# TopAY-Planner/TopAY

Hardware: AMD Instinct MI355X
Metric: trajectories/sec to L-BFGS convergence (benchmark_tables batch) at 1/2/4/8 GPU (higher is better)
Workload: dtype f64

## Files before the change

include/topay.h:

```cpp
#ifndef TOPAY_H
#define TOPAY_H

#include <stdint.h>

#ifdef __cplusplus
extern "C" {
#endif

typedef int topay_status;
enum {
  TOPAY_OK = 0,
  TOPAY_ERR_INVALID_ARG = -1,
  TOPAY_ERR_NO_DEVICE = -2,
  TOPAY_ERR_NO_MAP = -3,
  TOPAY_ERR_NO_TRAJ = -4,
  TOPAY_ERR_TOO_MANY_PIECES = -5,
  TOPAY_ERR_UNSUPPORTED = -6
};

enum {
  TOPAY_LBFGS_CONVERGENCE = 0,
  TOPAY_LBFGS_STOP = 1,
  TOPAY_LBFGS_CANCELED = 2,
  TOPAY_LBFGSERR_INVALID_FUNCVAL = -1012,
// ... 215 lines not shown

topay_status topay_set_latency_mode(topay_ctx* ctx, int mode);

typedef struct { char internal[128]; } topay_comm_id_t;
typedef struct {
  int scenario_id;
  int best_candidate;
  int status;
  int n_pieces;
  double cost;
  double duration;
} topay_record_t;
topay_status topay_comm_unique_id(topay_comm_id_t* id);
topay_status topay_comm_init(topay_ctx* ctx, const topay_comm_id_t* id, int world, int rank);
topay_status topay_comm_destroy(topay_ctx* ctx);
topay_status topay_scenario_records(topay_ctx* ctx, const int* scenario_of, int cap_records, topay_record_t* records, int* n_records,
                                    int* winner_index);
topay_status topay_gather_records(topay_ctx* ctx, const topay_record_t* mine, int n_mine, int per_rank, topay_record_t* all, int* n_valid);
topay_status topay_pack_records(const topay_record_t* mine, int n_mine, int per_rank, topay_record_t* block);
topay_status topay_unpack_records(const topay_record_t* gathered, int world, int per_rank, topay_record_t* all, int* n_valid);

topay_status topay_class_of(int n_pieces, int* waves, int* elements_per_thread, int* class_index);

topay_status topay_workspace_bytes(topay_ctx* ctx, unsigned long long* bytes);

topay_status topay_gate_timeouts(topay_ctx* ctx, int* n);

topay_status topay_last_kernel_ms(topay_ctx* ctx, double* ms, int* launches);
topay_status topay_last_helper_launches(topay_ctx* ctx, int* n);

#ifdef __cplusplus
}
#endif
#endif
```

topay_amd/csrc/topay_eval.h:

```cpp
#pragma once

#include <hip/hip_runtime.h>

#include "topay_math.h"
#include "topay_types.h"

#ifndef TOPAY_CPU_EMU
#define HIP_DYN_SHARED_DECL extern __shared__ double topay_lds[];
#endif

__constant__ DevParams g_P;
typedef const TOPAY_CST DevParams& dev_params_ref;
__device__ __forceinline__ dev_params_ref dev_params() {
#ifndef TOPAY_CPU_EMU
  const TOPAY_CST DevParams* p = (const TOPAY_CST DevParams*)&g_P;
  asm("" : "+s"(p));
  return *p;
#else
  return g_P;
#endif
}

#ifdef TOPAY_USE_SCHED_FENCE
#define TOPAY_SCHED_FENCE() __builtin_amdgcn_sched_barrier(0)
// ... 352 lines not shown
  gx = g0 * ri;
  dist = q.in ? dist : 0.0; gx = q.in ? gx : 0.0; gy = q.in ? gy : 0.0; gz = q.in ? gz : 0.0;
}

struct EvalCtx {
  int lane, N, rows, n;
  int tid, wave;
  lds_dp red;
  lds_dp adj;
  glb_dp coefg;
  int cl_in_lds;
  lds_dp cL;
  lds_dp Tp;
  glb_cdp hd, tl;
  int npass_lds;
  lds_dp gdT;
  lds_dp pcs;
  lds_dp gC;
  glb_dp sbuf;
  int sb_stride;
  glb_dp mstash;
  lds_dp pw;
  lds_dp X;
  glb_cdp x;
  glb_dp g;
  glb_dp lu;
  glb_cdp init_xy;
  double sx, sy, ex, ey;
  double lam0, lam1, rho0, rho1;
  double fxe0, fxe1;
  TOPAY_GLB long long* stamps;
  long long t_last;
};

__device__ __forceinline__ void fill_power_table(lds_dp pw, int lane) {
  for (int t = lane; t < 156; t += 64) {
    const int jj = t / 6, k = t - 6 * jj;
    double v = 1.0;
    for (int u = 0; u < k; u++) v *= (double)jj;
    pw[t] = v;
  }
}

#define BAND(i, j) band[((i) - (j) + 6) * rows + (j)]

#ifdef TOPAY_STAMPS
// ... 14 lines not shown
  } while (0)
#else
#define SUBSTAMP_BEGIN(C) do { } while (0)
#define SUBSTAMP_END(C, k) do { } while (0)
#endif

struct GradGate {
  bool always;
  bool has_early;
  double finit, thr , early ;
  bool early_ok;
  double skip_thr;
  __device__ __forceinline__ bool needs(double f) const {
    if (always) return true;
    if (isinf(f) || isnan(f)) return false;
    if (has_early && fabs(finit - f) / (fabs(finit) + 1.0) < early) return true;
    return !(f > thr);
  }
};

#define TOPAY_SWEEP_CHUNK 24
#define TOPAY_SWEEP_WCOLS 30
#define TOPAY_SWEEP_WIN (7 * TOPAY_SWEEP_WCOLS)
template <int MODE>
__device__ __forceinline__ void band_sweep(lds_dp v, bool owner, glb_cdp lu, lds_dp win, int rows, int lane) {
  constexpr bool FWD = (MODE == 0 || MODE == 2);
  constexpr bool SCALE = (MODE == 1 || MODE == 2);
  constexpr int D0 = (MODE == 0 || MODE == 3) ? 7 : 0;
  constexpr int CH = TOPAY_SWEEP_CHUNK, WC = TOPAY_SWEEP_WCOLS, WIN = TOPAY_SWEEP_WIN;
  constexpr int NEL = (SCALE ? 7 : 6) * WC;
  constexpr int NQ = (NEL + 63) / 64;
  double w[6];
  double x = 0.0;
#pragma unroll
  for (int t = 0; t < 6; t++) w[t] = 0.0;
  if (owner) {
    if (FWD) {
      x = v[0];
#pragma unroll
      for (int t = 0; t < 6; t++) w[t] = v[1 + t];
    } else {
      x = v[rows - 1];
#pragma unroll
      for (int t = 0; t < 6; t++) w[t] = v[rows - 2 - t];
    }
  }
  const int nchunk = (rows + CH - 1) / CH;
  auto chunk_clo = [&](int k) { return FWD ? CH * k : rows - 1 - CH * k - (WC - 1); };
  auto request = [&](int k, double (&q)[NQ]) {
    const int clo = chunk_clo(k);
#pragma unroll
    for (int u = 0; u < NQ; u++) {
      const int e = lane + 64 * u;
      const int r = e / WC, cc = e - r * WC;
      int c = clo + cc;
      c = c < 0 ? 0 : (c > rows - 1 ? rows - 1 : c);
      const int d = (r < 6 ? D0 + r : 13);
      q[u] = lu[(d < 14 ? d : 13) * rows + c];
    }
  };
  auto deposit = [&](int k, const double (&q)[NQ]) {
    lds_dp wb = win + (k & 1) * WIN;
#pragma unroll
    for (int u = 0; u < NQ; u++) {
      const int e = lane + 64 * u;
      if (e < NEL) wb[e] = q[u];
    }
  };
// ... 554 lines not shown
```

topay_amd/csrc/topay_eval_mw.h:

```cpp
#pragma once
#include "topay_eval.h"

namespace topay {

__device__ __forceinline__ void wg_lds_barrier() {
#ifndef TOPAY_CPU_EMU
  __builtin_amdgcn_fence(__ATOMIC_RELEASE, "workgroup", "local");
  __builtin_amdgcn_s_barrier();
  __builtin_amdgcn_fence(__ATOMIC_ACQUIRE, "workgroup", "local");
#else
  __syncthreads();
#endif
}

template <int NW>
__device__ __forceinline__ void wg_barrier() {
  if (NW == 1) lds_sync();
  else wg_lds_barrier();
}

template <int NW>
__device__ __forceinline__ void wg_global_barrier() {
  if (NW == 1) lds_sync();
  else __syncthreads();
// ... 21 lines not shown
  lds_dp r = red + (phase & 1) * 4;
  phase++;
  r[wave] = wm;
  wg_lds_barrier();
  double m = r[0] > r[1] ? r[0] : r[1];
  if (NW == 4) {
    const double m2 = r[2] > r[3] ? r[2] : r[3];
    m = m > m2 ? m : m2;
  }
  return m;
}

__host__ __device__ __forceinline__ int mw_pb_rows(int NW) { return NW == 1 ? 7 : 14; }
__host__ __device__ __forceinline__ int mw_npass(int Nmax) { return (TOPAY_EP * Nmax + 63) / 64; }
__host__ __device__ __forceinline__ int mw_red_doubles(int NW) { return NW > 1 ? 8 : 0; }
__host__ __device__ __forceinline__ int mw_misc_doubles(int Nmax, int NW) {
  return mw_red_doubles(NW) + 2 * mw_npass(Nmax) + (NW > 1 ? 2 * NW * 64 : 0) + NW;
}
__host__ __device__ __forceinline__ int lds_doubles_mw(int Nmax, int NW) {
  const int rows = 6 * Nmax;
  const int lu = 14 * rows, sw = 9 * rows + 26 * Nmax + mw_pb_rows(NW) * 64 * NW;
  return 5 * Nmax + Nmax + 4 * (Nmax + 1) + 156 + mw_misc_doubles(Nmax, NW) + (lu > sw ? lu : sw);
}
__device__ __forceinline__ void carve_mw(EvalCtx& C, lds_dp base, int Nmax, int NW) {
  const int rows = 6 * Nmax;
  lds_dp p = base;
  C.Tp = p; p += 5 * Nmax;
  C.gdT = p; p += Nmax;
  C.pcs = p; p += 4 * (Nmax + 1);
  C.pw = p; p += 156;
  C.red = p; p += mw_misc_doubles(Nmax, NW);
  C.cL = p;
  C.adj = C.cL;
  C.gC = C.adj;
  C.X = p + 9 * rows;
  C.npass_lds = mw_npass(Nmax);
}

template <int NW, int OCC>
__device__ __noinline__ void minco_generate_mw(EvalCtx& C) {
  constexpr int NT = 64 * NW;
  const lds_dp c_Tp = C.Tp;
  const lds_dp c_X = C.X;
  const lds_dp c_gdT = C.gdT;
  const glb_cdp c_hd = C.hd, c_tl = C.tl;
  const glb_dp c_lu = C.lu;
  const glb_cdp c_x = C.x;
  dev_params_ref P = dev_params();
  const int tid = C.tid, lane = C.lane, wave = __builtin_amdgcn_readfirstlane(C.wave);
  const int N = __builtin_amdgcn_readfirstlane(C.N), rows = __builtin_amdgcn_readfirstlane(C.rows);
  lds_dp cL = C.cL;
  lds_dp band = cL;
  lds_dp rdiag = cL + 13 * rows;
  glb_cdp Tau = c_x;
  glb_cdp Theta = c_x + N;
  glb_cdp Arc = c_x + 2 * N - 1;
  glb_cdp Vq = c_x + 3 * N - 1;

  const double tau_v = tid < N ? Tau[tid] : 0.0;
  constexpr int NI = 9;
  double inner_v[NI];
#pragma unroll
  for (int u = 0; u < NI; u++) {
    const int t = tid + NT * u;
    inner_v[u] = 0.0;
    if (t < 9 * (N - 1)) {
      const int i = t / 9, d = t - 9 * i;
      const int dq = d >= 2 ? d - 2 : 0;
      inner_v[u] = d == 0 ? Theta[i] : (d == 1 ? Arc[i] : Vq[i * 7 + dq]);
    }
  }
  double bc_v[6] = {0.0, 0.0, 0.0, 0.0, 0.0, 0.0};
  if (tid < 9) {
    const int d = tid;
    bc_v[0] = c_hd[0 * 9 + d]; bc_v[1] = c_hd[1 * 9 + d]; bc_v[2] = c_hd[2 * 9 + d];
    bc_v[3] = (d == 1) ? Arc[N - 1] : c_tl[0 * 9 + d];
// ... 40 lines not shown
  if (wave == 0) {
    const int t = lane / 7 + 1, u = lane - (lane / 7) * 7;
    const bool lane_in = lane < 42;
    const int o_kk = 6 * rows;
    const int o_ik = lane_in ? (t + 6) * rows : o_kk;
    const int o_ij = lane_in ? (t - u + 6) * rows + u : o_kk;
    const int o_kj = lane_in ? (6 - u) * rows + u : o_kk;
    for (int k = 0; k <= rows - 2; k++) {
      const int i = k + t, j = k + u;
      const bool act = lane_in && (i < rows) && (j < rows);
      double akk = band[o_kk + k], aik = band[o_ik + k], aij = band[o_ij + k], akj = band[o_kj + k];
      TOPAY_OPAQUE(aij); TOPAY_OPAQUE(akj);
      const double m = aik / akk;
      const double nv = (u == 0) ? m : (aij - m * akj);
      lds_sync();
      if (act) band[o_ij + k] = nv;
      lds_sync();
    }
  }
  wg_barrier<NW>();
  STAMP(C, 1);
  for (int t = tid; t < rows; t += NT) rdiag[t] = 1.0 / BAND(t, t);
  wg_barrier<NW>();
  for (int t = tid; t < 14 * rows; t += NT) c_lu[t] = band[t];
  if (NW == 1) lds_sync();
  else { wave_global_sync(); wg_barrier<NW>(); }
  for (int t = tid; t < 9 * rows; t += NT) cL[t] = 0.0;
  wg_barrier<NW>();
  if (tid < 9) {
    const int d = tid;
    cL[d * rows + 0] = bc_v[0];
    cL[d * rows + 1] = bc_v[1];
    cL[d * rows + 2] = bc_v[2];
    cL[d * rows + rows - 3] = bc_v[3];
    cL[d * rows + rows - 2] = bc_v[4];
    cL[d * rows + rows - 1] = bc_v[5];
  }
#pragma unroll
  for (int u = 0; u < NI; u++) {
    const int t = tid + NT * u;
    if (t < 9 * (N - 1)) {
      const int i = t / 9, d = t - 9 * i;
      const int dq = d >= 2 ? d - 2 : 0;
      cL[d * rows + 6 * i + 5] = d >= 2 ? sigmoidC2(inner_v[u], P.joint_pos_limit_max[dq]) : inner_v[u];
    }
  }
  wg_barrier<NW>();
  if (wave == 0) {
    const bool owner = lane < 9;
    const lds_dp mine = cL + (owner ? lane : 8) * rows;
    band_sweep<0>(mine, owner, (glb_cdp)c_lu, c_X, rows, lane);
    band_sweep<1>(mine, owner, (glb_cdp)c_lu, c_X, rows, lane);
  }
  C.cl_in_lds = 1;
  wg_barrier<NW>();
  STAMP(C, 2);
}

template <int STAGE, int RMAX, int NW, int OCC = 1>
__device__ __noinline__ TOPAY_CALLS_BIG_FUNCTIONS double eval_cost_grad_mw(EvalCtx& C, const TOPAY_GLB DevMap* mp, const GradGate gate) {
  constexpr int NT = 64 * NW;
  const lds_dp c_Tp = uniform_ptr(C.Tp);
  const lds_dp c_X = uniform_ptr(C.X);
  const double c_ex = uniform_f64(C.ex);
  const double c_ey = uniform_f64(C.ey);
  const glb_dp c_g = uniform_ptr(C.g);
  const lds_dp c_gdT = uniform_ptr(C.gdT);
  const glb_cdp c_init_xy = uniform_ptr(C.init_xy);
  const double c_lam0 = uniform_f64(C.lam0);
  const double c_lam1 = uniform_f64(C.lam1);
  const glb_dp c_lu = uniform_ptr(C.lu);
  const lds_dp c_pcs = uniform_ptr(C.pcs);
  const lds_dp c_pw = uniform_ptr(C.pw);
  const double c_rho0 = uniform_f64(C.rho0);
  const double c_rho1 = uniform_f64(C.rho1);
// ... 6 lines not shown

  dev_params_ref P = dev_params();
  int lane = C.lane, tid = C.tid;
  const int wave = __builtin_amdgcn_readfirstlane(C.wave);
  const int N = __builtin_amdgcn_readfirstlane(C.N), rows = __builtin_amdgcn_readfirstlane(C.rows);
  lds_cdp cL = uniform_ptr(C.cL);
  const glb_dp c_sbuf = uniform_ptr(C.sbuf);
  const glb_dp c_mstash = uniform_ptr(C.mstash);
  const int c_sbs = __builtin_amdgcn_readfirstlane(C.sb_stride);
  const double g_skip_thr = uniform_f64(gate.skip_thr);
  const bool g_early_ok = __builtin_amdgcn_readfirstlane(gate.early_ok ? 1 : 0) != 0;
  GradGate ugate;
  ugate.always = __builtin_amdgcn_readfirstlane(gate.always ? 1 : 0) != 0;
  ugate.has_early = __builtin_amdgcn_readfirstlane(gate.has_early ? 1 : 0) != 0;
  ugate.finit = uniform_f64(gate.finit); ugate.thr = uniform_f64(gate.thr); ugate.early = uniform_f64(gate.early);
  ugate.early_ok = g_early_ok; ugate.skip_thr = g_skip_thr;
  int rp = 0;
  const int npl = __builtin_amdgcn_readfirstlane(C.npass_lds);
  constexpr int RD = NW > 1 ? 8 : 0;
  const lds_dp ptot = c_red + RD;
  const lds_dp csr = c_red + RD + 2 * npl;
  TOPAY_LDS unsigned long long* jmask = (TOPAY_LDS unsigned long long*)(c_red + RD + 2 * npl + (NW > 1 ? 2 * NW * 64 : 0));
  constexpr int PBR = NW == 1 ? 7 : 14;
  minco_generate_mw<NW, OCC>(C);

  auto jerk_terms = [&](int i, double& e_out, double& gdT_out) __attribute__((always_inline)) {
    double w33 = 0, w43 = 0, w44 = 0, w53 = 0, w54 = 0, w55 = 0;
#pragma unroll
    for (int d = 0; d < 9; d++) {
      const double c3 = cL[d * rows + 6 * i + 3], c4 = cL[d * rows + 6 * i + 4], c5 = cL[d * rows + 6 * i + 5];
      const double e = P.energy_weights[d];
      w33 += (c3 * e) * c3; w43 += (c4 * e) * c3; w44 += (c4 * e) * c4;
      w53 += (c5 * e) * c3; w54 += (c5 * e) * c4; w55 += (c5 * e) * c5;
    }
    const double T1 = c_Tp[i], T2 = c_Tp[N + i], T3 = c_Tp[2 * N + i], T4 = c_Tp[3 * N + i], T5 = c_Tp[4 * N + i];
    e_out = 36.0 * w33 * T1 + 144.0 * w43 * T2 + 192.0 * w44 * T3 + 240.0 * w53 * T3 + 720.0 * w54 * T4 + 720.0 * w55 * T5;
    gdT_out = 36.0 * w33 + 288.0 * w43 * T1 + 576.0 * w44 * T2 + 720.0 * w53 * T2 + 2880.0 * w54 * T3 + 3600.0 * w55 * T4;
  };
  double jerk_e = 0.0;
  if (tid < N) {
    double unused_;
    jerk_terms(tid, jerk_e, unused_);
  }
  const double jerk_cost = wg_sum<NW>(c_red, rp, wave, jerk_e);

  lds_dp gxy = c_X;
// ... 79 lines not shown
        posy = c_sy + (carryy + py0);
      };
      geometry(lane);
      if (act && m == TOPAY_K) {
        c_pcs[2 * N + 2 * (i + 1)] = posx;
        c_pcs[2 * N + 2 * (i + 1) + 1] = posy;
      }
      if (!skip_body) {
        ManiOut mo;
        mo.gx = mo.gy = mo.gth = mo.cost = mo.gdT = 0.0;
        if (STAGE == 2) {
          mo = sample_mani<OCC>(cL, rows, i, j, e, act, step, half, posx, posy, mp, c_mstash, pbuf + lane);
          lane = fresh_lane_id(lane);
          tid = wave * 64 + lane;
          geometry(lane);
        }
        double gB[12], gdTs, gpx, gpy, cst;
        bool jva;
        sample_rest<STAGE>(P, cL, rows, i, j, step, half, posx, posy, mp, wM, wA, wD, mo, pbuf + lane, gB, gdTs, gpx, gpy, jva, cst);
        if (act) {
          cst_out = cst;
          gxy[2 * e] = gpx;
          gxy[2 * e + 1] = gpy;
          glb_dp sb = c_sbuf + e;
          const int ss = c_sbs;
#pragma unroll
          for (int v = 0; v < 5; v++) sb[v * ss] = gB[v];
          sb[5 * ss] = gdTs;
          if (STAGE == 2) {
#pragma unroll
            for (int v = 0; v < 7; v++) sb[(6 + v) * ss] = gB[5 + v];
            sb[13 * ss] = jva ? 1.0 : 0.0;
          }
        }
      }
    }
    lds_dp cs = csr + (k & 1) * (NW * 64);
    if (NW > 1) {
      cs[wave * 64 + lane] = cst_out;
      wg_barrier<NW>();
    }
#pragma unroll
    for (int q = 0; q < NW; q++) {
      const int p2 = k * NW + q;
      if (p2 < npass) {
        cost_pen += NW > 1 ? cs[q * 64 + lane] : cst_out;
        if (STAGE == 2 && g_early_ok && !skip_body && p2 + 1 < npass) {
          const double partial = jerk_cost + wave_sum(cost_pen) + time_cost;
          if (partial > g_skip_thr && partial <= 1.79769313486231570e308) {
            skip_body = true;
            f_skip = partial;
          }
        }
      }
    }
// ... 74 lines not shown
  for (int r = 0; r < RMAX; r++) {
    a0[r] = 0.0;
    a1[r] = 0.0;
#pragma unroll
    for (int q = 0; q < 7; q++) aq[r][q] = 0.0;
    rbh[r][0] = rbh[r][1] = rbh[r][2] = 0.0;
    if (ract[r]) {
      const double hs = c_Tp[rpiece[r]] / TOPAY_K / 2.0;
      basis_k(rk[r], hs, rbh[r][0], rbh[r][1], rbh[r][2]);
    }
  }
  constexpr int NV = (STAGE == 2) ? 13 : 6;
  if constexpr (NW == 1) {
    for (int pass = 0; pass < npass; pass++) {
      const int e = pass * 64 + lane;
      const bool act = e < NE;
      const int i = act ? e / TOPAY_EP : N - 1;
      const int m = act ? e - TOPAY_EP * i : 0;
      const int j = 2 * m;
      const double step = c_Tp[i] / TOPAY_K, half = step / 2.0;
      bool jva = false;
      double rawq[7];
      {
        glb_cdp sb = c_sbuf + (act ? e : NE - 1);
        const int ss = c_sbs;
        double raw[14];
#pragma unroll
        for (int v = 0; v < ((STAGE == 2) ? 14 : 6); v++) raw[v] = sb[v * ss];
#pragma unroll
        for (int v = 0; v < 6; v++) pbuf[v * 64 + lane] = act ? raw[v] : 0.0;
#pragma unroll
        for (int v = 0; v < 7; v++) rawq[v] = (STAGE == 2 && act) ? raw[6 + v] : 0.0;
        if (STAGE == 2) jva = act && raw[13] != 0.0;
      }
      lds_sync();
#pragma unroll
      for (int r = 0; r < RMAX; r++) {
        if (ract[r]) {
          const int pi = rpiece[r];
          const double h0 = rbh[r][0], h1 = rbh[r][1], h2 = rbh[r][2];
          const int k0 = rk[r], k1 = rk[r] >= 1 ? rk[r] - 1 : 0, k2 = rk[r] >= 2 ? rk[r] - 2 : 0;
          const int e_lo = max(TOPAY_EP * pi, pass * 64), e_hi = min(min(TOPAY_EP * pi + TOPAY_EP, pass * 64 + 64), NE);
          double gt = 0.0;
          constexpr int CH = 3;
          for (int c0 = e_lo; c0 < e_hi; c0 += CH) {
            double pb[CH][6], t0[CH], t1[CH], t2[CH];
#pragma unroll
            for (int u = 0; u < CH; u++) {
              const int ee = (c0 + u < e_hi) ? c0 + u : e_hi - 1;
              const int l = ee - pass * 64, mm = ee - TOPAY_EP * pi;
              lds_cdp pj = c_pw + 12 * mm;
// ... 401 lines not shown
          const double e = P.energy_weights[d];
          if (kk == 5) jg = 240.0 * c3 * e * T3 + 720.0 * c4 * e * T4 + 1440.0 * c5 * e * T5;
          else if (kk == 4) jg = 144.0 * c3 * e * T2 + 384.0 * c4 * e * T3 + 720.0 * c5 * e * T4;
          else jg = 72.0 * c3 * e * T1 + 144.0 * c4 * e * T2 + 240.0 * c5 * e * T3;
        }
        tot[r][d] = jg + (d == 0 ? a0[r] : (d == 1 ? a1[r] : aq[r][d >= 2 ? d - 2 : 0]));
      }
    }
  }
  for (int t = tid; t < 9 * rows; t += NT) c_coefg[t] = cL[t];
  C.cl_in_lds = 0;
  wg_global_barrier<NW>();
#pragma unroll
  for (int r = 0; r < RMAX; r++) {
    if (ract[r]) {
#pragma unroll
      for (int d = 0; d < 9; d++) c_adj[d * rows + rrow[r]] = tot[r][d];
    }
  }
  wg_barrier<NW>();
  if (wave == 0) {
    const bool owner = lane < 9;
    const lds_dp mine = c_adj + (owner ? lane : 8) * rows;
    band_sweep<2>(mine, owner, (glb_cdp)c_lu, c_X, rows, lane);
    band_sweep<3>(mine, owner, (glb_cdp)c_lu, c_X, rows, lane);
  }
  wg_barrier<NW>();
  STAMP(C, 7);
#pragma unroll
  for (int r = 0; r < RMAX; r++) {
    if (ract[r]) {
      const int row = rrow[r];
      int pi, br;
      bool use = true;
      if (row >= rows - 3) { pi = N - 1; br = 10 + (row - (rows - 3)); }
      else if (row < 3) { use = false; pi = 0; br = 0; }
      else { pi = (row - 3) / 6; br = (row - 3) - 6 * pi; }
      double part = 0.0;
      if (use) {
        const double T1 = c_Tp[pi], T2 = c_Tp[N + pi], T3 = c_Tp[2 * N + pi], T4 = c_Tp[3 * N + pi];
#pragma unroll
        for (int d = 0; d < 9; d++) {
          glb_cdp cg = c_coefg + d * rows + 6 * pi;
          const double c1 = cg[1], c2 = cg[2], c3 = cg[3], c4 = cg[4], c5 = cg[5];
          double b;
          if (br == 0) b = -(24.0 * c4 + 120.0 * T1 * c5);
          else if (br == 1) b = -120.0 * c5;
          else if (br == 2 || br == 3 || br == 10) b = -(c1 + 2.0 * T1 * c2 + 3.0 * T2 * c3 + 4.0 * T3 * c4 + 5.0 * T4 * c5);
// ... 36 lines not shown
```

topay_amd/csrc/topay_hip.hip:

```cpp
#include <hip/hip_runtime.h>

#include <algorithm>
#include <cstdio>
#include <cstdint>
#include <cstring>
#include <numeric>
#include <cstdlib>
#include <chrono>
#include <cmath>
#include <mutex>
#include <thread>
#include <string>
#include <vector>
#include <dlfcn.h>

#include "topay_solve.h"
#include "topay_feas.h"
#include "topay_edt.h"
#include "topay_front.h"
#include "topay_mcrrt.h"
#include "topay_jps.h"
#include "topay_topo.h"
#include "topay_yaml.h"

// ... 94 lines not shown
      if (atoi(e) == 4) {
        if (w4 == 4) t[4] = {42, 2, 4, k_solve2w4, k_eval2w4, 2};
        if (w5 == 4) t[5] = {64, 2, 4, k_solve2w4, k_eval2w4, 2};
        t[6] = {128, 3, 4, k_solve3w4, k_eval3w4, 2};
      }
    }
#endif
    return t;
  }();
  return tab;
}
static const int kLdsDoublesPerCU = 160 * 1024 / 8;
static size_t class_lds_bytes(const ClassDef& cd, int nm) {
  int d = lds_doubles_mw(nm, cd.nw);
  if (const char* e = exp_env("TOPAY_LDS_PAD")) {
    for (const char* q = e; q && *q;) {
      int mn = 0, add = 0;
      if (sscanf(q, "%d:%d", &mn, &add) == 2 && mn == cd.max_n) d += add;
      q = strchr(q, ',');
      if (q) q++;
    }
  }
  return (size_t)(d + 8 + 40 + (cd.helpers ? TOPAY_CMD_DOUBLES : 0)) * sizeof(double);
}

__attribute__((constructor)) static void topay_request_hw_queues() { setenv("GPU_MAX_HW_QUEUES", "24", 0); }
struct topay_ctx;
static std::mutex g_issue_mutex;
static std::mutex g_registry_mutex;
static std::vector<topay_ctx*> g_contexts;

static topay_ctx* g_last_issued = nullptr;

struct topay_ctx {
  int device = 0;
  topay_params_t hp;
  DevParams dp;
  hipStream_t stream = nullptr;
  hipEvent_t ev0 = nullptr, ev1 = nullptr;
  std::vector<DevMap> hmaps = std::vector<DevMap>(TOPAY_MAX_MAPS);
  std::vector<DevBuf> map2d = std::vector<DevBuf>(TOPAY_MAX_MAPS), map3d = std::vector<DevBuf>(TOPAY_MAX_MAPS);
  std::vector<DevBuf> map2d_inf = std::vector<DevBuf>(TOPAY_MAX_MAPS), map2d_crit = std::vector<DevBuf>(TOPAY_MAX_MAPS);
  struct MapArena { DevBuf buf; int first = 0, n = 0; };
  std::vector<MapArena> map_arenas;
  DevBuf dmaps;
  std::vector<char> have_map = std::vector<char>(TOPAY_MAX_MAPS, 0);
// ... 10 lines not shown
  std::vector<int> cls[NBUCKET];
  hipStream_t bstream[NBUCKET] = {nullptr};
  hipEvent_t bevent[NBUCKET] = {nullptr};
  hipEvent_t bstart = nullptr;
  bool pending = false;
  int* h_started = nullptr;
  int n_launched = 0;
  int n_gate = 0;
  bool gate = true;
  bool gate_in_solve = true;
  int latency_mode = 0;
  bool gate_done = false;
  std::vector<int> h_group;
  int n_groups = 0, cancel_budget = 0;
  DevBuf group_id, group_tau, interrupted;
  int* h_cancel = nullptr;
  void* comm = nullptr;
  int comm_world = 0, comm_rank = 0;
  hipStream_t comm_stream = nullptr;
  DevBuf comm_send, comm_recv;
  int gate_timeouts = 0;
  bool persistent = true;
  bool steal = true;
  int simd_slots = 1024;
  double occ2_gain = 1.7;
  DevBuf qnext;
  DevBuf mc_i, mc_d, mc_k, mc_rs, mc_in;
  int mc_n = 0, mc_node_cap = 0;
  DevBuf tp_i, tp_d, tp_raw, tp_pts, tp_io;
  int tp_n = 0, tp_pt_cap = 0, tp_nbuf = 0;
  topay_topo_params_t tp_P;
  DevBuf paths, path_off, path_len, bvel, bacc, scratch;
  DevBuf N, s1_past, map_id, head, tail, start_xy, goal_xy, init_xy, x0;
  DevBuf x, work, hist_s, hist_y, hist_ys, hist_alpha, lu;
  DevBuf success, cost, stats, xyerr, coef, T, knots, alm, fout, order, trace, elapsed, startus, hwid, sbuf, mstash, feas_cseq, feas_tk, feas_report, feas_flags, edt_occ, edt_tmp1, edt_tmp2, edt_v, edt_z, edt_out2, edt_out3, pb_io;
  float last_edt_ms = 0.f;
  int trace_cap = 0;
  DevBatch db;
  bool have_traj = false, solved = false;
  double last_ms = 0.0;
  int last_launches = 0, last_helper_launches = 0;
};

static void make_dev_params(const topay_params_t& p, DevParams& d) {
  memset(&d, 0, sizeof(d));
  d.relu_mu = p.relu_mu;
// ... 180 lines not shown
  make_dev_params(*params, c->dp);
  const topay_status st = create_device_state(c, device);
  if (st != TOPAY_OK) { topay_destroy(c); return st; }
  {
    std::lock_guard<std::mutex> lk(g_registry_mutex);
    g_contexts.push_back(c);
  }
  *out = c;
  return TOPAY_OK;
}

static topay_status create_device_state(topay_ctx* c, int device) {
  HIPCHK(hipStreamCreateWithFlags(&c->stream, hipStreamNonBlocking));
  HIPCHK(hipEventCreate(&c->ev0));
  HIPCHK(hipEventCreate(&c->ev1));
  HIPCHK(hipEventCreate(&c->bstart));
  for (int k = 0; k < topay_ctx::NBUCKET; k++) {
    if (k >= topay_ctx::NBUCKET - 2) c->bstream[k] = c->stream;
    else HIPCHK(hipStreamCreateWithFlags(&c->bstream[k], hipStreamNonBlocking));
    HIPCHK(hipEventCreate(&c->bevent[k]));
  }
  {
    { const char* se = getenv("TOPAY_STEAL"); c->steal = !(se && se[0] == '0'); }
    const char* pe = getenv("TOPAY_PERSISTENT");
    c->persistent = !(pe && pe[0] == '0');
    hipDeviceProp_t prop;
    HIPCHK(hipGetDeviceProperties(&prop, device));
    c->simd_slots = 4 * prop.multiProcessorCount;
    if (const char* og = exp_env("TOPAY_OCC2_GAIN")) c->occ2_gain = std::max(0.5, atof(og));
    {
      const char* rs = exp_env("TOPAY_RESERVE_SLOTS");
      const int reserve = rs ? atoi(rs) : 0;
      if (reserve > 0 && reserve < c->simd_slots / 2) c->simd_slots -= reserve;
    }
  }
  {
    const char* g = exp_env("TOPAY_DISPATCH_GATE");
    c->gate = !(g && g[0] == '0');
    void* hp = nullptr;
    HIPCHK(hipHostMalloc(&hp, 64, hipHostMallocMapped | hipHostMallocCoherent));
    c->h_started = (int*)hp;
    c->h_started[0] = 0;
    c->h_cancel = c->h_started + 8;
    c->h_cancel[0] = 0;
    { const char* ge = exp_env("TOPAY_GATE_IN_SOLVE"); c->gate_in_solve = !(ge && ge[0] == '0'); }
  }
// ... 613 lines not shown
static int steal_floor(int k) {
  const ClassDef* ct = class_table();
  int lo = k;
  while (lo > 0 && ct[lo - 1].nw == ct[k].nw && ct[lo - 1].snw() == ct[k].snw() && ((lo - 1 >= kBigFirst) == (k >= kBigFirst))) lo--;
  return lo;
}

template <bool EVAL, typename... Args>
static topay_status launch_classes(topay_ctx* c, bool persistent, Args... args) {
  const ClassDef* ct = class_table();
  int launches = 0, helper_launches = 0, off = 0;
  topay_status ps = push_params(c);
  if (ps != TOPAY_OK) return ps;
  HIPCHK(set_kernel_attributes(c->device));
  int slots = 0;
  if (persistent) {
    if (c->qnext.ensure(sizeof(int) * topay_ctx::NBUCKET) != TOPAY_OK) return TOPAY_ERR_NO_DEVICE;
    HIPCHK(hipMemsetAsync(c->qnext.p, 0, sizeof(int) * topay_ctx::NBUCKET, c->stream));
    slots = c->simd_slots;
  }
  int pgrid[topay_ctx::NBUCKET] = {0}, nmk[topay_ctx::NBUCKET] = {0};
  for (int k = 0; k < topay_ctx::NBUCKET; k++) {
    for (int b : c->cls[k]) nmk[k] = std::max(nmk[k], c->hN[b]);
    if (persistent && c->steal)
      for (int k2 = steal_floor(k); k2 < k; k2++)
        for (int b : c->cls[k2]) nmk[k] = std::max(nmk[k], c->hN[b]);
  }
  if (persistent) {
    static const double over = [] { const char* e = exp_env("TOPAY_OVERSUBSCRIBE"); return e ? atof(e) : 1.08; }();
    compute_grids(c, nmk, slots / 4.0 * over, pgrid);
  }
  HIPCHK(hipEventRecord(c->bstart, c->stream));
  for (int k = topay_ctx::NBUCKET - 1; k >= 0; k--) {
    const std::vector<int>& v = c->cls[k];
    const int nk = (int)v.size();
    if (nk == 0) continue;
    const int nm = nmk[k];
    DevBatch d = c->db;
    d.order = c->db.order + off;
    int grid = nk;
    if (persistent) {
      d.order = c->db.order;
      d.queue_next = c->qnext.as<int>();
      d.queue_class = k;
      d.queue_lowest = c->steal ? steal_floor(k) : k;
      int o2 = 0;
      for (int kk = topay_ctx::NBUCKET - 1; kk >= 0; kk--) {
        d.queue_off[kk] = o2;
        d.queue_count[kk] = (int)c->cls[kk].size();
        o2 += d.queue_count[kk];
      }
      grid = pgrid[k];
    }
    off += nk;
    const bool lat = !EVAL && ct[k].lat && (c->latency_mode == 2 || (c->latency_mode == 1 && c->B <= c->simd_slots));
    size_t lds = class_lds_bytes(ct[k], nm);
    if (lat) {
      lds = (size_t)(lds_doubles_mw(nm, kLatWaves) + 8 + 40 + TOPAY_CMD_DOUBLES) * sizeof(double);
      grid = nk;
    }
    if (k == topay_ctx::NBUCKET - 2 && !c->cls[topay_ctx::NBUCKET - 1].empty() && c->bstream[k] == c->stream)
      HIPCHK(hipStreamCreateWithFlags(&c->bstream[k], hipStreamNonBlocking));
    hipStream_t st = c->bstream[k];
    if (st != c->stream) HIPCHK(hipStreamWaitEvent(st, c->bstart, 0));
    if constexpr (EVAL) hipLaunchKernelGGL(ct[k].eval, dim3(grid), dim3(64 * ct[k].nw), lds, st, d, (const DevMap*)c->dmaps.p, args..., nm);
    else if (lat) { hipLaunchKernelGGL(ct[k].lat, dim3(grid), dim3(64 * kLatWaves), lds, st, d, (const DevMap*)c->dmaps.p, nm); helper_launches++; }
    else hipLaunchKernelGGL(ct[k].solve, dim3(grid), dim3(64 * ct[k].nw), lds, st, d, (const DevMap*)c->dmaps.p, nm);
    HIPCHK(hipGetLastError());
    if (st != c->stream) HIPCHK(hipEventRecord(c->bevent[k], st));
    launches++;
  }
  for (int k = 0; k < topay_ctx::NBUCKET; k++)
    if (!c->cls[k].empty() && c->bstream[k] != c->stream) HIPCHK(hipStreamWaitEvent(c->stream, c->bevent[k], 0));
  c->last_launches = launches;
  c->last_helper_launches = helper_launches;
  return TOPAY_OK;
}


// ... 991 lines not shown
  return false;
}

static topay_status eval_one(topay_ctx* c, int stage, int i, const double* x, const double* alm_lambda, const double* alm_rho,
                             double* f, double* g, double* final_xy_error, bool commit, int force_nw = 0) {
  if (!c || !c->have_traj) return TOPAY_ERR_NO_TRAJ;
  if (i < 0 || i >= c->B || (stage != 1 && stage != 2) || !x) return TOPAY_ERR_INVALID_ARG;
  HIPCHK(hipSetDevice(c->device));
  if (c->pending) { topay_status ws = topay_synchronize(c); if (ws != TOPAY_OK) return ws; }
  const int N = c->hN[i], nn = 10 * N - 8;
  if (N == 0) return TOPAY_ERR_TOO_MANY_PIECES;
  HIPCHK(memcpy_sync(c, c->x.as<double>() + c->h_noff[i], x, (size_t)nn * 8, hipMemcpyHostToDevice));
  double alm[4] = {alm_lambda ? alm_lambda[0] : c->hp.alm_init_lambda[0], alm_lambda ? alm_lambda[1] : c->hp.alm_init_lambda[1],
                   alm_rho ? alm_rho[0] : c->hp.alm_init_rho[0], alm_rho ? alm_rho[1] : c->hp.alm_init_rho[1]};
  HIPCHK(memcpy_sync(c, c->alm.as<double>() + (size_t)i * 4, alm, 32, hipMemcpyHostToDevice));
  ScopedDevBuf tmp;
  topay_status s = tmp.ensure(4);
  if (s != TOPAY_OK) return s;
  HIPCHK(memcpy_sync(c, tmp.p, &i, 4, hipMemcpyHostToDevice));
  DevBatch d = c->db;
  d.order = tmp.as<int>();
  ClassDef cd = class_table()[bucket_of(N)];
  if (force_nw > 0 && !class_for_waves(N, force_nw, cd)) { set_err("no kernel with that many waves holds this candidate"); return TOPAY_ERR_UNSUPPORTED; }
  const size_t lds = class_lds_bytes(cd, N);
  if ((s = push_params(c)) != TOPAY_OK) return s;
  HIPCHK(set_kernel_attributes(c->device));
  if (force_nw > 0) HIPCHK(hipFuncSetAttribute((const void*)cd.eval, hipFuncAttributeMaxDynamicSharedMemorySize, kLdsDoublesPerCU * 8));
  hipLaunchKernelGGL(cd.eval, dim3(1), dim3(64 * cd.nw), lds, c->stream, d, (const DevMap*)c->dmaps.p, stage | (commit ? 16 : 0), 1, N);
  HIPCHK(hipGetLastError());
  HIPCHK(hipStreamSynchronize(c->stream));
  tmp.release();
  if (f) HIPCHK(memcpy_sync(c, f, c->fout.as<double>() + i, 8, hipMemcpyDeviceToHost));
  if (g) HIPCHK(memcpy_sync(c, g, c->work.as<double>() + 4 * c->h_noff[i], (size_t)nn * 8, hipMemcpyDeviceToHost));
  if (final_xy_error) HIPCHK(memcpy_sync(c, final_xy_error, c->xyerr.as<double>() + 2 * i, 16, hipMemcpyDeviceToHost));
  return TOPAY_OK;
}
}

extern "C" {
topay_status topay_eval(topay_ctx* c, int stage, int i, const double* x, const double* alm_lambda, const double* alm_rho,
                        double* f, double* g, double* final_xy_error) {
  return eval_one(c, stage, i, x, alm_lambda, alm_rho, f, g, final_xy_error, false);
}

topay_status topay_eval_waves(topay_ctx* c, int stage, int i, int waves, const double* x, const double* alm_lambda, const double* alm_rho,
                              double* f, double* g, double* final_xy_error) {
  if (waves != 1 && waves != 2 && waves != 4) return TOPAY_ERR_INVALID_ARG;
// ... 273 lines not shown
  topay_status s;
  if ((s = c->comm_send.ensure(bytes)) != TOPAY_OK || (s = c->comm_recv.ensure(bytes * c->comm_world)) != TOPAY_OK) return s;
  std::vector<topay_record_t> pad((size_t)per_rank);
  (void)topay_pack_records(mine, n_mine, per_rank, pad.data());
  HIPCHK(hipMemcpyAsync(c->comm_send.p, pad.data(), bytes, hipMemcpyHostToDevice, c->comm_stream));
  const int rc = a->AllGather(c->comm_send.p, c->comm_recv.p, bytes, 0 , c->comm, c->comm_stream);
  if (rc != 0) return rccl_fail("ncclAllGather", rc);
  std::vector<topay_record_t> got((size_t)per_rank * c->comm_world);
  HIPCHK(hipMemcpyAsync(got.data(), c->comm_recv.p, bytes * c->comm_world, hipMemcpyDeviceToHost, c->comm_stream));
  HIPCHK(hipStreamSynchronize(c->comm_stream));
  return topay_unpack_records(got.data(), c->comm_world, per_rank, all, n_valid);
}

topay_status topay_class_of(int n_pieces, int* waves, int* elements_per_thread, int* class_index) {
  if (n_pieces <= 0 || n_pieces > TOPAY_MAX_N) return TOPAY_ERR_TOO_MANY_PIECES;
  const int k = bucket_of(n_pieces);
  const ClassDef& cd = class_table()[k];
  if (waves) *waves = cd.snw();
  if (elements_per_thread) *elements_per_thread = 2 * cd.srmax();
  if (class_index) *class_index = k;
  return TOPAY_OK;
}

topay_status topay_workspace_bytes(topay_ctx* c, unsigned long long* bytes) {
  if (!c || !bytes) return TOPAY_ERR_INVALID_ARG;
  *bytes = (unsigned long long)c->workspace_bytes;
  return TOPAY_OK;
}

topay_status topay_gate_timeouts(topay_ctx* c, int* n) {
  if (!c || !n) return TOPAY_ERR_INVALID_ARG;
  *n = c->gate_timeouts;
  return TOPAY_OK;
}

topay_status topay_last_kernel_ms(topay_ctx* c, double* ms, int* launches) {
  if (!c) return TOPAY_ERR_INVALID_ARG;
  if (ms) *ms = c->last_ms;
  if (launches) *launches = c->last_launches;
  return TOPAY_OK;
}

topay_status topay_last_helper_launches(topay_ctx* c, int* n) {
  if (!c || !n) return TOPAY_ERR_INVALID_ARG;
  *n = c->last_helper_launches;
  return TOPAY_OK;
// ... 11 lines not shown
```

topay_amd/csrc/topay_kernels.h:

```cpp
#pragma once
#include <hip/hip_runtime.h>

#include "topay_solve.h"
#include "topay_feas.h"
#include "topay_edt.h"
#include "topay_front.h"
#include "topay_mcrrt.h"
#include "topay_jps.h"

using namespace topay;

#ifndef TOPAY_CPU_EMU
extern __shared__ double topay_lds[];
#define TOPAY_LDS_PTR ((lds_dp)topay_lds)
#else
#define TOPAY_LDS_PTR ((lds_dp)hip_emu::S().dyn_smem)
#endif

__global__ void k_init(DevBatch Bt, const double* paths, const long long* path_off, const int* path_len,
                       const double* bvel, const double* bacc, double* scratch, int scratch_stride, int maxN, int stride_n) {
  const int b = blockIdx.x * blockDim.x + threadIdx.x;
  if (b >= Bt.B) return;
  init_one(g_P, paths + path_off[b] * 10, path_len[b], bvel + (size_t)b * 20, bacc + (size_t)b * 20,
           scratch + (size_t)b * scratch_stride, maxN, Bt.N + b, Bt.s1_past + b, Bt.head + (size_t)b * 27,
// ... 2 lines not shown
}

__device__ __forceinline__ long long uniform_i64(long long v) {
  const unsigned lo = (unsigned)__builtin_amdgcn_readfirstlane((int)(v & 0xffffffffLL)), hi = (unsigned)__builtin_amdgcn_readfirstlane((int)(v >> 32));
  return (long long)(((unsigned long long)hi << 32) | lo);
}

template <int NW>
__host__ __device__ __forceinline__ int eval_lds_doubles(int Nmax_lds) {
  return lds_doubles_mw(Nmax_lds, NW);
}

template <int RMAX, int NW>
__device__ __forceinline__ void load_ctx(EvalCtx& C, const DevBatch& Bt, int b, int Nmax_lds) {
  constexpr int NT = 64 * NW;
  C.tid = threadIdx.x;
  C.lane = threadIdx.x & 63;
  C.wave = threadIdx.x >> 6;
  C.N = __builtin_amdgcn_readfirstlane(Bt.N[b]);
  C.rows = 6 * C.N;
  C.n = 10 * C.N - 8;
  C.red = nullptr; C.adj = nullptr; C.cl_in_lds = 1;
  carve_mw(C, TOPAY_LDS_PTR, Nmax_lds, NW);
  fill_power_table(C.pw, C.lane);
  C.hd = (glb_cdp)(Bt.head + (size_t)b * 27);
  C.tl = (glb_cdp)(Bt.tail + (size_t)b * 27);
  const long long po = uniform_i64(Bt.poff[b]);
  C.lu = (glb_dp)(Bt.lu + 84 * po);
  C.sb_stride = TOPAY_EP * C.N;
  C.sbuf = (glb_dp)(Bt.sbuf + 14 * TOPAY_EP * po);
  C.mstash = (glb_dp)(Bt.mstash + 36 * TOPAY_EP * po);
  C.coefg = (glb_dp)(Bt.coef + 54 * po);
  C.init_xy = (glb_cdp)(Bt.init_xy + (size_t)b * 2 * TOPAY_MAX_N);
  C.sx = Bt.start_xy[2 * b]; C.sy = Bt.start_xy[2 * b + 1];
  C.ex = Bt.goal_xy[2 * b];  C.ey = Bt.goal_xy[2 * b + 1];
  C.fxe0 = 0.0; C.fxe1 = 0.0;
  C.stamps = nullptr;
  C.t_last = 0;
#ifdef TOPAY_STAMPS
  if (Bt.trace && Bt.trace_cap >= 32) C.stamps = (TOPAY_GLB long long*)(Bt.trace + (size_t)b * Bt.trace_cap) + 8;
  C.t_last = (long long)__builtin_amdgcn_s_memtime();
#endif
}

template <int NW>
__device__ __forceinline__ void store_result(const EvalCtx& C, const DevBatch& Bt, int b) {
// ... 341 lines not shown
```

topay_amd/csrc/topay_types.h:

```cpp
#pragma once
#include "../../include/topay.h"

#define TOPAY_K 12
#define TOPAY_SP 25
#define TOPAY_EP 13
#define TOPAY_NSPH 12
#define TOPAY_MAX_N 170
#define TOPAY_NBUCKET 7
#define TOPAY_WAVE 64

#ifndef TOPAY_LDS
#define TOPAY_LDS __attribute__((address_space(3)))
#endif
#ifndef TOPAY_GLB
#define TOPAY_GLB __attribute__((address_space(1)))
#endif
#ifndef TOPAY_CST
#if defined(__HIP_DEVICE_COMPILE__)
#define TOPAY_CST __attribute__((address_space(4)))
#else
#define TOPAY_CST
#endif
#endif
typedef TOPAY_LDS double* lds_dp;
// ... 71 lines not shown
  double* x0;
  double* x;
  double* work;
  double* hist_s;
  double* hist_y;
  double* hist_ys;
  double* hist_alpha;
  double* lu;
  int* success;
  double* cost;
  int* stats;
  double* xyerr;
  double* coef;
  double* T;
  double* knots;
  double* alm;
  double* fout;
  double* sbuf;
  double* mstash;
  double* start_us;
  int* queue_next;
  int queue_count[TOPAY_NBUCKET], queue_off[TOPAY_NBUCKET], queue_class;
  int queue_lowest;
  int gate_in_solve;
  int* gate_truncated;
  int* feas_flags;
  double* feas_report;
  const int* group_id;
  int* group_tau;
  int cancel_budget;
  const int* cancel_flag;
  int* interrupted;
  int* started;
  int gate_maxN;
  int* hw_id;
  double* elapsed_us;
  const int* order;
  double* trace;
  int trace_cap;
};
```

Baseline: 7554.

## Keep LU band and per-pass stash in spare LDS when occupancy allows

Adds an LDS planning step that works out how much shared memory per workgroup is left over at the current occupancy. It uses that spare space to keep the banded LU factor resident, so the triangular sweeps read it from LDS instead of streaming windows from global memory. It also parks per-pass gradient scratch in LDS instead of the global sbuf. This only applies to single-wave classes, and it requests more dynamic LDS per launch. The plan is meant to stay within the same workgroups-per-CU, but the sweep order changes to a register-blocked serial loop, and a mode environment variable and an N-overflow check are added.

```diff
diff --git a/include/topay.h b/include/topay.h
--- a/include/topay.h
+++ b/include/topay.h
@@ -261,6 +261,8 @@
 
 topay_status topay_class_of(int n_pieces, int* waves, int* elements_per_thread, int* class_index);
 
+topay_status topay_lds_plan(int class_index, int n_longest, int mode, int* out);
+
 topay_status topay_workspace_bytes(topay_ctx* ctx, unsigned long long* bytes);
 
 topay_status topay_gate_timeouts(topay_ctx* ctx, int* n);
diff --git a/topay_amd/csrc/topay_eval.h b/topay_amd/csrc/topay_eval.h
--- a/topay_amd/csrc/topay_eval.h
+++ b/topay_amd/csrc/topay_eval.h
@@ -398,6 +398,10 @@
   glb_dp mstash;
   lds_dp pw;
   lds_dp X;
+  lds_dp rband;
+  lds_dp park;
+  int band_res;
+  int park1, park2;
   glb_cdp x;
   glb_dp g;
   glb_dp lu;
@@ -458,7 +462,7 @@
 #define TOPAY_SWEEP_CHUNK 24
 #define TOPAY_SWEEP_WCOLS 30
 #define TOPAY_SWEEP_WIN (7 * TOPAY_SWEEP_WCOLS)
-template <int MODE>
+template <int MODE, bool RESIDENT = false>
 __device__ __forceinline__ void band_sweep(lds_dp v, bool owner, glb_cdp lu, lds_dp win, int rows, int lane) {
   constexpr bool FWD = (MODE == 0 || MODE == 2);
   constexpr bool SCALE = (MODE == 1 || MODE == 2);
@@ -480,6 +484,49 @@
 #pragma unroll
       for (int t = 0; t < 6; t++) w[t] = v[rows - 2 - t];
     }
+  }
+  if constexpr (RESIDENT) {
+    if (owner) {
+      lds_cdp band = win;
+#pragma unroll 1
+      for (int b0 = 0; b0 < rows; b0 += 6) {
+        double cf[6][6], sc[6], nw[6];
+#pragma unroll
+        for (int u = 0; u < 6; u++) {
+          const int j = FWD ? b0 + u : rows - 1 - (b0 + u);
+#pragma unroll
+          for (int t = 1; t <= 6; t++) {
+            int idx;
+            if (MODE == 0) idx = (6 + t) * rows + j;
+            else if (MODE == 1) idx = (6 - t) * rows + j;
+            else if (MODE == 2) idx = (6 - t) * rows + j + t;
+            else idx = (6 + t) * rows + j - t;
+            cf[u][t - 1] = band[idx];
+          }
+          if (SCALE) sc[u] = band[13 * rows + j];
+          int in = FWD ? j + 7 : j - 7;
+          in = in < 0 ? 0 : (in > rows - 1 ? rows - 1 : in);
+          nw[u] = v[in];
+        }
+        double xo[6];
+#pragma unroll
+        for (int u = 0; u < 6; u++) {
+          const double xs = SCALE ? x * sc[u] : x;
+          xo[u] = xs;
+#pragma unroll
+          for (int t = 0; t < 6; t++) w[(u + t) % 6] -= cf[u][t] * xs;
+          x = w[u % 6];
+          w[u % 6] = nw[u];
+        }
+#pragma unroll
+        for (int u = 0; u < 6; u++) {
+          const int j = FWD ? b0 + u : rows - 1 - (b0 + u);
+          v[j] = xo[u];
+        }
+      }
+    }
+    lds_sync();
+    return;
   }
   const int nchunk = (rows + CH - 1) / CH;
   auto chunk_clo = [&](int k) { return FWD ? CH * k : rows - 1 - CH * k - (WC - 1); };
diff --git a/topay_amd/csrc/topay_eval_mw.h b/topay_amd/csrc/topay_eval_mw.h
--- a/topay_amd/csrc/topay_eval_mw.h
+++ b/topay_amd/csrc/topay_eval_mw.h
@@ -67,6 +67,44 @@
   const int lu = 14 * rows, sw = 9 * rows + 26 * Nmax + mw_pb_rows(NW) * 64 * NW;
   return 5 * Nmax + Nmax + 4 * (Nmax + 1) + 156 + mw_misc_doubles(Nmax, NW) + (lu > sw ? lu : sw);
 }
+__host__ __device__ __forceinline__ int lds_cl_offset_mw(int Nmax, int NW) {
+  return 5 * Nmax + Nmax + 4 * (Nmax + 1) + 156 + mw_misc_doubles(Nmax, NW);
+}
+__host__ __device__ __forceinline__ int lds_x_doubles_mw(int Nmax, int NW) { return 26 * Nmax + mw_pb_rows(NW) * 64 * NW; }
+struct LdsPlan {
+  int band_off, park_off, park1, park2;
+  int total_doubles;
+};
+#define TOPAY_LDS_CU_DOUBLES (160 * 1024 / 8)
+#define TOPAY_LDS_BUDGET_QUANTUM 320
+__host__ __device__ __forceinline__ int lds_wgs_per_cu(int doubles, int wg_cap) {
+  const int w = TOPAY_LDS_CU_DOUBLES / doubles;
+  return w < wg_cap ? w : wg_cap;
+}
+__host__ __device__ __forceinline__ LdsPlan lds_plan_mw(int Nmax, int NW, int base_doubles, int wg_cap, int mode) {
+  LdsPlan p;
+  p.band_off = 0; p.park_off = 0; p.park1 = 0; p.park2 = 0; p.total_doubles = base_doubles;
+  if (mode == 0 || NW != 1 || wg_cap < 1 || base_doubles > TOPAY_LDS_CU_DOUBLES) return p;
+  const int wgs = lds_wgs_per_cu(base_doubles, wg_cap);
+  const int budget = (TOPAY_LDS_CU_DOUBLES / wgs) / TOPAY_LDS_BUDGET_QUANTUM * TOPAY_LDS_BUDGET_QUANTUM;
+  int spare = budget - base_doubles;
+  const int band = 14 * 6 * Nmax, npass = mw_npass(Nmax);
+  int at = base_doubles;
+  auto take_parks = [&]() {
+    int p2 = spare > 0 ? spare / (14 * 64) : 0, p1 = spare > 0 ? spare / (6 * 64) : 0;
+    p.park2 = p2 < npass ? p2 : npass;
+    p.park1 = p1 < npass ? p1 : npass;
+    const int used = p.park2 * 14 * 64 > p.park1 * 6 * 64 ? p.park2 * 14 * 64 : p.park1 * 6 * 64;
+    if (used > 0) { p.park_off = at; at += used; spare -= used; }
+  };
+  auto take_band = [&]() {
+    if (spare >= band) { p.band_off = at; at += band; spare -= band; }
+  };
+  if (mode == 2) { take_parks(); take_band(); }
+  else { take_band(); take_parks(); }
+  p.total_doubles = at;
+  return p;
+}
 __device__ __forceinline__ void carve_mw(EvalCtx& C, lds_dp base, int Nmax, int NW) {
   const int rows = 6 * Nmax;
   lds_dp p = base;
@@ -74,12 +112,14 @@
   C.gdT = p; p += Nmax;
   C.pcs = p; p += 4 * (Nmax + 1);
   C.pw = p; p += 156;
-  C.red = p; p += mw_misc_doubles(Nmax, NW);
+  C.red = p;
+  p = base + lds_cl_offset_mw(Nmax, NW);
   C.cL = p;
   C.adj = C.cL;
   C.gC = C.adj;
   C.X = p + 9 * rows;
   C.npass_lds = mw_npass(Nmax);
+  C.rband = base; C.park = base; C.band_res = 0; C.park1 = 0; C.park2 = 0;
 }
 
 template <int NW, int OCC>
@@ -95,8 +135,9 @@
   const int tid = C.tid, lane = C.lane, wave = __builtin_amdgcn_readfirstlane(C.wave);
   const int N = __builtin_amdgcn_readfirstlane(C.N), rows = __builtin_amdgcn_readfirstlane(C.rows);
   lds_dp cL = C.cL;
-  lds_dp band = cL;
-  lds_dp rdiag = cL + 13 * rows;
+  const bool resident = NW == 1 && __builtin_amdgcn_readfirstlane(C.band_res) != 0;
+  lds_dp band = resident ? C.rband : cL;
+  lds_dp rdiag = band + 13 * rows;
   glb_cdp Tau = c_x;
   glb_cdp Theta = c_x + N;
   glb_cdp Arc = c_x + 2 * N - 1;
@@ -183,9 +224,11 @@
   STAMP(C, 1);
   for (int t = tid; t < rows; t += NT) rdiag[t] = 1.0 / BAND(t, t);
   wg_barrier<NW>();
-  for (int t = tid; t < 14 * rows; t += NT) c_lu[t] = band[t];
-  if (NW == 1) lds_sync();
-  else { wave_global_sync(); wg_barrier<NW>(); }
+  if (!resident) {
+    for (int t = tid; t < 14 * rows; t += NT) c_lu[t] = band[t];
+    if (NW == 1) lds_sync();
+    else { wave_global_sync(); wg_barrier<NW>(); }
+  }
   for (int t = tid; t < 9 * rows; t += NT) cL[t] = 0.0;
   wg_barrier<NW>();
   if (tid < 9) {
@@ -210,8 +253,13 @@
   if (wave == 0) {
     const bool owner = lane < 9;
     const lds_dp mine = cL + (owner ? lane : 8) * rows;
-    band_sweep<0>(mine, owner, (glb_cdp)c_lu, c_X, rows, lane);
-    band_sweep<1>(mine, owner, (glb_cdp)c_lu, c_X, rows, lane);
+    if (NW == 1 && resident) {
+      band_sweep<0, true>(mine, owner, (glb_cdp)c_lu, band, rows, lane);
+      band_sweep<1, true>(mine, owner, (glb_cdp)c_lu, band, rows, lane);
+    } else {
+      band_sweep<0>(mine, owner, (glb_cdp)c_lu, c_X, rows, lane);
+      band_sweep<1>(mine, owner, (glb_cdp)c_lu, c_X, rows, lane);
+    }
   }
   C.cl_in_lds = 1;
   wg_barrier<NW>();
@@ -264,6 +312,9 @@
   const lds_dp csr = c_red + RD + 2 * npl;
   TOPAY_LDS unsigned long long* jmask = (TOPAY_LDS unsigned long long*)(c_red + RD + 2 * npl + (NW > 1 ? 2 * NW * 64 : 0));
   constexpr int PBR = NW == 1 ? 7 : 14;
+  constexpr int PKR = (STAGE == 2) ? 14 : 6;
+  const lds_dp c_park = uniform_ptr(C.park);
+  const int npark = NW == 1 ? __builtin_amdgcn_readfirstlane(STAGE == 2 ? C.park2 : C.park1) : 0;
   minco_generate_mw<NW, OCC>(C);
 
   auto jerk_terms = [&](int i, double& e_out, double& gdT_out) __attribute__((always_inline)) {
@@ -389,15 +440,27 @@
           cst_out = cst;
           gxy[2 * e] = gpx;
           gxy[2 * e + 1] = gpy;
-          glb_dp sb = c_sbuf + e;
-          const int ss = c_sbs;
-#pragma unroll
-          for (int v = 0; v < 5; v++) sb[v * ss] = gB[v];
-          sb[5 * ss] = gdTs;
-          if (STAGE == 2) {
-#pragma unroll
-            for (int v = 0; v < 7; v++) sb[(6 + v) * ss] = gB[5 + v];
-            sb[13 * ss] = jva ? 1.0 : 0.0;
+          if (NW == 1 && pass < npark) {
+            lds_dp pk = c_park + pass * (PKR * 64) + lane;
+#pragma unroll
+            for (int v = 0; v < 5; v++) pk[v * 64] = gB[v];
+            pk[5 * 64] = gdTs;
+            if (STAGE == 2) {
+#pragma unroll
+              for (int v = 0; v < 7; v++) pk[(6 + v) * 64] = gB[5 + v];
+              pk[13 * 64] = jva ? 1.0 : 0.0;
+            }
+          } else {
+            glb_dp sb = c_sbuf + e;
+            const int ss = c_sbs;
+#pragma unroll
+            for (int v = 0; v < 5; v++) sb[v * ss] = gB[v];
+            sb[5 * ss] = gdTs;
+            if (STAGE == 2) {
+#pragma unroll
+              for (int v = 0; v < 7; v++) sb[(6 + v) * ss] = gB[5 + v];
+              sb[13 * ss] = jva ? 1.0 : 0.0;
+            }
           }
         }
       }
@@ -518,11 +581,17 @@
       bool jva = false;
       double rawq[7];
       {
-        glb_cdp sb = c_sbuf + (act ? e : NE - 1);
-        const int ss = c_sbs;
         double raw[14];
-#pragma unroll
-        for (int v = 0; v < ((STAGE == 2) ? 14 : 6); v++) raw[v] = sb[v * ss];
+        if (pass < npark) {
+          lds_cdp pk = c_park + pass * (PKR * 64) + lane;
+#pragma unroll
+          for (int v = 0; v < PKR; v++) raw[v] = pk[v * 64];
+        } else {
+          glb_cdp sb = c_sbuf + (act ? e : NE - 1);
+          const int ss = c_sbs;
+#pragma unroll
+          for (int v = 0; v < PKR; v++) raw[v] = sb[v * ss];
+        }
 #pragma unroll
         for (int v = 0; v < 6; v++) pbuf[v * 64 + lane] = act ? raw[v] : 0.0;
 #pragma unroll
@@ -970,8 +1039,14 @@
   if (wave == 0) {
     const bool owner = lane < 9;
     const lds_dp mine = c_adj + (owner ? lane : 8) * rows;
-    band_sweep<2>(mine, owner, (glb_cdp)c_lu, c_X, rows, lane);
-    band_sweep<3>(mine, owner, (glb_cdp)c_lu, c_X, rows, lane);
+    if (NW == 1 && __builtin_amdgcn_readfirstlane(C.band_res) != 0) {
+      const lds_dp rband = uniform_ptr(C.rband);
+      band_sweep<2, true>(mine, owner, (glb_cdp)c_lu, rband, rows, lane);
+      band_sweep<3, true>(mine, owner, (glb_cdp)c_lu, rband, rows, lane);
+    } else {
+      band_sweep<2>(mine, owner, (glb_cdp)c_lu, c_X, rows, lane);
+      band_sweep<3>(mine, owner, (glb_cdp)c_lu, c_X, rows, lane);
+    }
   }
   wg_barrier<NW>();
   STAMP(C, 7);
diff --git a/topay_amd/csrc/topay_hip.hip b/topay_amd/csrc/topay_hip.hip
--- a/topay_amd/csrc/topay_hip.hip
+++ b/topay_amd/csrc/topay_hip.hip
@@ -140,6 +140,13 @@
     }
   }
   return (size_t)(d + 8 + 40 + (cd.helpers ? TOPAY_CMD_DOUBLES : 0)) * sizeof(double);
+}
+static LdsPlan class_lds_plan(const ClassDef& cd, int nm, int mode) {
+  const int base = (int)(class_lds_bytes(cd, nm) / sizeof(double));
+  return lds_plan_mw(nm, cd.helpers ? 0 : cd.nw, base, 4 * cd.occ / cd.nw, mode);
+}
+static void apply_lds_plan(DevBatch& d, const LdsPlan& p) {
+  d.lds_band_off = p.band_off; d.lds_park_off = p.park_off; d.lds_park1 = p.park1; d.lds_park2 = p.park2;
 }
 
 __attribute__((constructor)) static void topay_request_hw_queues() { setenv("GPU_MAX_HW_QUEUES", "24", 0); }
@@ -196,6 +203,7 @@
   int gate_timeouts = 0;
   bool persistent = true;
   bool steal = true;
+  int lds_mode = 1;
   int simd_slots = 1024;
   double occ2_gain = 1.7;
   DevBuf qnext;
@@ -422,6 +430,7 @@
   }
   {
     { const char* se = getenv("TOPAY_STEAL"); c->steal = !(se && se[0] == '0'); }
+    { const char* le = getenv("TOPAY_LDS_RESIDENT"); c->lds_mode = (le && le[0] >= '0' && le[0] <= '2') ? le[0] - '0' : 1; }
     const char* pe = getenv("TOPAY_PERSISTENT");
     c->persistent = !(pe && pe[0] == '0');
     hipDeviceProp_t prop;
@@ -1081,6 +1090,10 @@
   int pgrid[topay_ctx::NBUCKET] = {0}, nmk[topay_ctx::NBUCKET] = {0};
   for (int k = 0; k < topay_ctx::NBUCKET; k++) {
     for (int b : c->cls[k]) nmk[k] = std::max(nmk[k], c->hN[b]);
+    if (nmk[k] > ct[k].max_n) {
+      set_err("a candidate has more pieces than the kernel of its launch class holds");
+      return TOPAY_ERR_UNSUPPORTED;
+    }
     if (persistent && c->steal)
       for (int k2 = steal_floor(k); k2 < k; k2++)
         for (int b : c->cls[k2]) nmk[k] = std::max(nmk[k], c->hN[b]);
@@ -1114,6 +1127,11 @@
     off += nk;
     const bool lat = !EVAL && ct[k].lat && (c->latency_mode == 2 || (c->latency_mode == 1 && c->B <= c->simd_slots));
     size_t lds = class_lds_bytes(ct[k], nm);
+    if (!lat) {
+      const LdsPlan plan = class_lds_plan(ct[k], nm, c->lds_mode);
+      apply_lds_plan(d, plan);
+      lds = (size_t)plan.total_doubles * sizeof(double);
+    }
     if (lat) {
       lds = (size_t)(lds_doubles_mw(nm, kLatWaves) + 8 + 40 + TOPAY_CMD_DOUBLES) * sizeof(double);
       grid = nk;
@@ -2151,7 +2169,9 @@
   d.order = tmp.as<int>();
   ClassDef cd = class_table()[bucket_of(N)];
   if (force_nw > 0 && !class_for_waves(N, force_nw, cd)) { set_err("no kernel with that many waves holds this candidate"); return TOPAY_ERR_UNSUPPORTED; }
-  const size_t lds = class_lds_bytes(cd, N);
+  const LdsPlan plan = class_lds_plan(cd, N, c->lds_mode);
+  apply_lds_plan(d, plan);
+  const size_t lds = (size_t)plan.total_doubles * sizeof(double);
   if ((s = push_params(c)) != TOPAY_OK) return s;
   HIPCHK(set_kernel_attributes(c->device));
   if (force_nw > 0) HIPCHK(hipFuncSetAttribute((const void*)cd.eval, hipFuncAttributeMaxDynamicSharedMemorySize, kLdsDoublesPerCU * 8));
@@ -2471,6 +2491,26 @@
   return TOPAY_OK;
 }
 
+topay_status topay_lds_plan(int class_index, int n_longest, int mode, int* out) {
+  if (!out || class_index < 0 || class_index >= TOPAY_NBUCKET || mode < 0 || mode > 2) return TOPAY_ERR_INVALID_ARG;
+  const ClassDef& cd = class_table()[class_index];
+  if (n_longest <= 0 || n_longest > cd.max_n) return TOPAY_ERR_TOO_MANY_PIECES;
+  const LdsPlan p = class_lds_plan(cd, n_longest, mode);
+  const int rows = 6 * n_longest, eval_doubles = lds_doubles_mw(n_longest, cd.nw);
+  out[0] = (int)(class_lds_bytes(cd, n_longest) / sizeof(double));
+  out[1] = p.total_doubles;
+  out[2] = p.band_off; out[3] = p.band_off ? 14 * rows : 0;
+  out[4] = p.park_off; out[5] = std::max(p.park1 * 6 * 64, p.park2 * 14 * 64);
+  out[6] = p.park1; out[7] = p.park2;
+  out[8] = 4 * cd.occ / cd.nw;
+  out[9] = 0; out[10] = 5 * n_longest;
+  out[11] = lds_cl_offset_mw(n_longest, cd.nw); out[12] = 9 * rows;
+  out[13] = out[11] + 9 * rows; out[14] = lds_x_doubles_mw(n_longest, cd.nw);
+  out[15] = eval_doubles; out[16] = out[0] - eval_doubles;
+  out[17] = mw_npass(n_longest);
+  return TOPAY_OK;
+}
+
 topay_status topay_workspace_bytes(topay_ctx* c, unsigned long long* bytes) {
   if (!c || !bytes) return TOPAY_ERR_INVALID_ARG;
   *bytes = (unsigned long long)c->workspace_bytes;
diff --git a/topay_amd/csrc/topay_kernels.h b/topay_amd/csrc/topay_kernels.h
--- a/topay_amd/csrc/topay_kernels.h
+++ b/topay_amd/csrc/topay_kernels.h
@@ -48,6 +48,13 @@
   C.n = 10 * C.N - 8;
   C.red = nullptr; C.adj = nullptr; C.cl_in_lds = 1;
   carve_mw(C, TOPAY_LDS_PTR, Nmax_lds, NW);
+  if (NW == 1) {
+    C.band_res = Bt.lds_band_off != 0;
+    C.rband = TOPAY_LDS_PTR + Bt.lds_band_off;
+    C.park = TOPAY_LDS_PTR + Bt.lds_park_off;
+    C.park1 = Bt.lds_park1;
+    C.park2 = Bt.lds_park2;
+  }
   fill_power_table(C.pw, C.lane);
   C.hd = (glb_cdp)(Bt.head + (size_t)b * 27);
   C.tl = (glb_cdp)(Bt.tail + (size_t)b * 27);
diff --git a/topay_amd/csrc/topay_types.h b/topay_amd/csrc/topay_types.h
--- a/topay_amd/csrc/topay_types.h
+++ b/topay_amd/csrc/topay_types.h
@@ -117,6 +117,7 @@
   int* queue_next;
   int queue_count[TOPAY_NBUCKET], queue_off[TOPAY_NBUCKET], queue_class;
   int queue_lowest;
+  int lds_band_off = 0, lds_park_off = 0, lds_park1 = 0, lds_park2 = 0;
   int gate_in_solve;
   int* gate_truncated;
   int* feas_flags;
```

New measurement: 7533 (median of 2 runs). About the same (-0.3%).
